# locuslab/icnn

Measured on AMD Instinct MI355X. Metric: inner-solves/sec (batch x iters), n=159 K=10, higher is better.
Workload: dtype f32 PICNN / f64 dual solve

## Files before the change

icnn_amd/_lib.py:

```python
import ctypes as C
import os

import torch

HERE = os.path.dirname(os.path.abspath(__file__))
LIB_PATH = os.path.join(HERE, "csrc", "libicnn_be.so")
if os.environ.get("ICNN_BE_LIB"):
    LIB_PATH = os.path.abspath(os.environ["ICNN_BE_LIB"])

ABI_VERSION = 12
MAX_LAYERS = 8
MAX_SLOTS = 31
MAX_ITERS = 64
MAX_ROUNDS = 128
VARIANT = {"dual": 0, "rl": 1, "pdipm": 2}
CUT_F32, CUT_F64 = 0, 1
ST_SINGULAR, ST_NONFINITE, ST_OVERFLOW, ST_UNFINISHED = 1, 2, 4, 8
ST_ERROR_MASK = ST_SINGULAR | ST_NONFINITE | ST_UNFINISHED | ST_OVERFLOW
FLAG_NO_CYCLE_SHORTCUT = 1
FLAG_TIME_SLICE = 2
FLAG_LOCKSTEP = 4
FLAG_TWO_KERNELS = 8
FLAG_PERSISTENT = 16
FLAG_F64_ENERGY = 32
FLAG_GLOBAL_BUNDLE = 64
FLAG_WAVE_PER_SAMPLE = 128
FLAG_MFMA_CONTRACTION = 256
FLAG_GENERIC_SHAPE = 512
SHAPE_INSTANCES = ["generic", "bibtex_kt16", "bibtex_kt32_grouped"]
LOSS = {"xent": 0, "mse": 1}
PATHS = ["ROWS", "TILE", "TILE_BUDGETED_THEN_ROWS", "ROUNDS_LOCKSTEP", "ROUNDS_SLICED_THEN_ROWS", "ROUNDS_SLICED_EXTRA"]
ADAM_KERNELS = ["NONE", "ROWS", "TILE"]
DUAL_KERNELS = ["small", "body", "wide"]
ERRORS = {-1: "ICNN_BE_EINVAL (bad argument)", -2: "ICNN_BE_ELIMIT (size beyond a compiled-in limit)",
          -3: "ICNN_BE_ELAUNCH (HIP launch failed)"}

EXPORTS = [
    "icnn_be_abi_version", "icnn_be_last_hip_error", "icnn_be_struct_size", "icnn_be_dual_lds_bytes", "icnn_be_bundle_capacity", "icnn_be_scratch_bytes",
    "icnn_be_state_init",
    "icnn_be_dual_step", "icnn_be_fc_pack_floats", "icnn_be_fc_pack", "icnn_be_fc_fg",
    "icnn_be_solve_fc", "icnn_be_solve_fc_reset", "icnn_be_conv_pack_floats", "icnn_be_conv_work_floats", "icnn_be_conv_pack", "icnn_be_conv_fg", "icnn_be_solve_conv",
    "icnn_be_implicit_feed", "icnn_be_export_active", "icnn_be_adam_workspace_bytes", "icnn_be_adam_fc", "icnn_be_adam_fc_obs",
    "icnn_be_adam_fc_each", "icnn_be_debug_adam_each_plan",
    "icnn_be_fc_context_work_floats", "icnn_be_fc_context", "icnn_be_fc_context_stage", "icnn_be_fc_context_norm", "icnn_be_fc_clamp",
    "icnn_be_conv_context_work_floats", "icnn_be_conv_context", "icnn_be_conv_clamp",
    "icnn_be_debug_profile", "icnn_be_debug_profile_fc", "icnn_be_debug_profile_conv", "icnn_be_debug_profile_phases",
    "icnn_be_debug_fast_math", "icnn_be_debug_trace", "icnn_be_debug_solve_plan", "icnn_be_debug_adam_plan", "icnn_be_debug_dual_plan",
    "icnn_be_debug_shape_instance", "icnn_be_debug_fc_deal",
    "icnn_be_fc_grad_floats", "icnn_be_fc_surrogate_grad_work_floats", "icnn_be_fc_surrogate_grad",
    "icnn_be_conv_grad_floats", "icnn_be_conv_surrogate_grad_work_floats", "icnn_be_conv_surrogate_grad",
    "icnn_be_fc_context_bn_work_floats", "icnn_be_fc_context_bn", "icnn_be_conv_context_bn_work_floats", "icnn_be_conv_context_bn",
# ... 639 lines not shown
```

icnn_amd/csrc/be_dual_dev.h:

```cpp
#pragma once
#include <hip/hip_runtime.h>
#include <math.h>
#include <type_traits>

#include "be_common.h"
#include "be_kernels.h"
#include "icnn_be.h"

namespace icnn_be {

namespace {

constexpr double BOUND_EPS = 1e-12;
constexpr double ARMIJO_ALPHA = 1e-5;
constexpr double GRAD_TOL = 1e-10;
constexpr double TINY = 1e-10;
constexpr double CYCLE_TOL = 1e-13;
constexpr double NOISE_TOL = 1e-10;
constexpr int NOISE_T0 = 12;
constexpr int ACCEL_T0 = 24;
constexpr int ACCEL_GAP = 6;
constexpr double ACCEL_NEG_RESID = 1e-10;
constexpr double ACCEL_D2MAX = 1e-3;
constexpr double ACCEL_RMAX = 0.98;
// ... 465 lines not shown
    }
#pragma unroll
    for (int p = KT - 1; p >= 0; --p) {
        if (p < k && ((fmask >> p) & 1ull)) {
            const double x = bcast(M[KT] * rinv, p);
            M[KT] = lane == p ? x : (lane < p ? M[KT] - M[p] * x : M[KT]);
        }
    }
    return StepResult{is_free ? M[KT] : 0.0, 1};
}

template <int I, int N, typename F>
__device__ __forceinline__ void static_for(F &&f) {
    if constexpr (I < N) {
        f(std::integral_constant<int, I>{});
        static_for<I + 1, N>(f);
    }
}
template <int P>
__device__ __forceinline__ double row_bcast(double v) {
    return __builtin_amdgcn_update_dpp(0.0, v, 0x150 + P, 0xf, 0xf, true);
}

template <int KS>
__device__ __noinline__ int inertia_not_above_dpp(const double *Hm_, int HP, int k, double mu) {
    static_assert(KS <= 16, "row broadcasts stay inside one 16-lane row");
    const int lane = lane_id();
    lds_cdouble *Hm = (lds_cdouble *)Hm_;
    HP = uni(HP); k = uni(k); mu = uni(mu);
    double M[KS];
#pragma unroll
    for (int j = 0; j < KS; ++j) M[j] = Hm[(lane < k ? lane : 0) * HP + (j < k ? j : 0)];
#pragma unroll
    for (int j = 0; j < KS; ++j) pin(M[j]);
#pragma unroll
    for (int j = 0; j < KS; ++j)
        M[j] = (lane < k && j < k) ? M[j] - (j == lane ? mu : 0.0) : (j == lane ? 1.0 : 0.0);
    double dp = 1.0;
    static_for<0, KS>([&](auto P) {
        constexpr int p = decltype(P)::value;
        const double d = row_bcast<p>(M[p]);
        dp = lane == p ? d : dp;
        const double nf = lane > p ? -(M[p] * rcp_nr(d)) : 0.0;
        static_for<p + 1, KS>([&](auto J) {
            constexpr int j = decltype(J)::value;
            M[j] = __builtin_fma(nf, row_bcast<p>(M[j]), M[j]);
        });
    });
    const unsigned long long nonpos = __ballot(lane < k && !(dp > 0.0));
    const unsigned long long zero = __ballot(lane < k && dp == 0.0);
    if (zero) {
        const int p0 = __builtin_ctzll(zero);
        return __popcll(nonpos & ((2ull << p0) - 1ull)) + (k - p0 - 1);
    }
    return __popcll(nonpos);
}

template <int KS, bool TRI = false>
__device__ __noinline__ StepResult newton_step_dpp(const double *Hm_, int HP, int k, int piv,
                                                   unsigned long long fmask, bool is_free, double g0) {
    static_assert(KS <= 16, "row broadcasts stay inside one 16-lane row");
    const int lane = lane_id();
    lds_cdouble *Hm = (lds_cdouble *)Hm_;
    HP = uni(HP); k = uni(k); piv = uni(piv); fmask = uni(fmask);
    double M[KS + 1];
    const int rl = lane < k ? lane : 0;
    auto at = [&](int i, int j) -> int {
        if (!TRI) return i * HP + j;
        const int c = i > j ? i : j, r = i > j ? j : i;
        return c * (c + 1) / 2 + r;
    };
    double h_ip = Hm[at(rl, piv)], h_pp = Hm[at(piv, piv)];
#pragma unroll
    for (int j = 0; j < KS; ++j) M[j] = Hm[at(rl, j < k ? j : 0)];
    pin(h_ip);
    pin(h_pp);
#pragma unroll
    for (int j = 0; j < KS; ++j) pin(M[j]);
    static_for<0, KS>([&](auto J) {
        constexpr int j = decltype(J)::value;
        double hv = ((M[j] - row_bcast<j>(h_ip)) - h_ip) + h_pp;
        pin(hv);
        const bool use = j < k && is_free && ((fmask >> j) & 1ull);
        M[j] = use ? hv : (j == lane ? 1.0 : 0.0);
    });
    M[KS] = is_free ? -g0 : 0.0;
    double rinv = 1.0;
    bool bad = false;
    static_for<0, KS>([&](auto P) {
        constexpr int p = decltype(P)::value;
        const double d = row_bcast<p>(M[p]);
        bad |= !(d != 0.0);
        const double inv = rcp_nr(d);
        rinv = lane == p ? inv : rinv;
        const double nf = lane > p ? -(M[p] * inv) : 0.0;
        static_for<p + 1, KS + 1>([&](auto J) {
            constexpr int j = decltype(J)::value;
            M[j] = __builtin_fma(nf, row_bcast<p>(M[j]), M[j]);
        });
        __builtin_amdgcn_sched_barrier(0);
    });
    if (__ballot(bad) & 0xffffull) return StepResult{0.0, 0};
    static_for<0, KS>([&](auto Q) {
        constexpr int p = KS - 1 - decltype(Q)::value;
        const double x = row_bcast<p>(M[KS] * rinv);
        M[KS] = lane == p ? x : (lane < p ? __builtin_fma(-M[p], x, M[KS]) : M[KS]);
    });
    return StepResult{is_free ? M[KS] : 0.0, 1};
}

__device__ __forceinline__ void swap16(double &x, double &y) {
    const auto lo = __builtin_amdgcn_permlane16_swap((unsigned)__double2loint(x), (unsigned)__double2loint(y), false, false);
    const auto hi = __builtin_amdgcn_permlane16_swap((unsigned)__double2hiint(x), (unsigned)__double2hiint(y), false, false);
    x = __hiloint2double((int)hi[0], (int)lo[0]);
    y = __hiloint2double((int)hi[1], (int)lo[1]);
}
__device__ __forceinline__ void swap32(double &x, double &y) {
    const auto lo = __builtin_amdgcn_permlane32_swap((unsigned)__double2loint(x), (unsigned)__double2loint(y), false, false);
    const auto hi = __builtin_amdgcn_permlane32_swap((unsigned)__double2hiint(x), (unsigned)__double2hiint(y), false, false);
    x = __hiloint2double((int)hi[0], (int)lo[0]);
    y = __hiloint2double((int)hi[1], (int)lo[1]);
}
template <int Q>
__device__ __forceinline__ double quarter_bcast(double v) {
    double a = v, b = v;
    swap16(a, b);
    double c = (Q & 1) ? b : a, d = c;
    swap32(c, d);
    return Q < 2 ? c : d;
}
__device__ __forceinline__ void quarter_gather(double v, double (&out)[4]) {
    double a = v, b = v;
// ... 123 lines not shown
            nf1 = quarter_bcast<qp>(i1 > p ? -(M1[sp] * inv) : 0.0);
        }
        static_for<sp, NS>([&](auto S) {
            constexpr int s = decltype(S)::value;
            const double pr = row_bcast<rp>(upper ? M1[s] : M0[s]);
            if constexpr (!upper) M0[s] = __builtin_fma(nf0, pr, M0[s]);
            M1[s] = __builtin_fma(nf1, pr, M1[s]);
        });
        __builtin_amdgcn_sched_barrier(0);
    });
    const bool own = (r & 3) == q;
    auto fold = [](unsigned long long m) -> unsigned { return (unsigned)((m | (m >> 16) | (m >> 32) | (m >> 48)) & 0xffffull); };
    unsigned nonpos = fold(__ballot(own && !(dp0 > 0.0))) | (fold(__ballot(own && !(dp1 > 0.0))) << 16);
    unsigned zero = fold(__ballot(own && dp0 == 0.0)) | (fold(__ballot(own && dp1 == 0.0)) << 16);
    const unsigned live = k >= 32 ? 0xffffffffu : ((1u << k) - 1u);
    nonpos &= live; zero &= live;
    if (zero) {
        const int p0 = __builtin_ctz(zero);
        return __popc(nonpos & ((2u << p0) - 1u)) + (k - p0 - 1);
    }
    return __popc(nonpos);
}

template <int KT>
__device__ __forceinline__ int inertia_not_above(const double *Hm, int HP, int k, double mu) {
    if (k <= 4) return inertia_not_above_dpp<4>(Hm, HP, k, mu);
    if (k <= 6) return inertia_not_above_dpp<6>(Hm, HP, k, mu);
    if (k <= 8) return inertia_not_above_dpp<8>(Hm, HP, k, mu);
    if (k <= 10) return inertia_not_above_dpp<10>(Hm, HP, k, mu);
    if (k <= 12) return inertia_not_above_dpp<12>(Hm, HP, k, mu);
    if (KT == 16 || k <= 16) return inertia_not_above_dpp<16>(Hm, HP, k, mu);
    if constexpr (KT > 16) {
        if (k <= 20) return inertia_not_above_2d<20>(Hm, HP, k, mu);
        if (k <= 24) return inertia_not_above_2d<24>(Hm, HP, k, mu);
        return inertia_not_above_2d<32>(Hm, HP, k, mu);
    }
    return 0;
}
__device__ __forceinline__ StepResult newton_step_tri(const double *P, int k, int piv, unsigned long long fmask, bool is_free,
                                                      double g0) {
    if (k <= 4) return newton_step_dpp<4, true>(P, 0, k, piv, fmask, is_free, g0);
    if (k <= 6) return newton_step_dpp<6, true>(P, 0, k, piv, fmask, is_free, g0);
    return newton_step_dpp<8, true>(P, 0, k, piv, fmask, is_free, g0);
}
template <int KT>
__device__ __forceinline__ StepResult newton_step(const double *Hm, int HP, int k, int piv, unsigned long long fmask,
                                                  bool is_free, double g0) {
    if (k <= 4) return newton_step_dpp<4>(Hm, HP, k, piv, fmask, is_free, g0);
    if (k <= 6) return newton_step_dpp<6>(Hm, HP, k, piv, fmask, is_free, g0);
    if (k <= 8) return newton_step_dpp<8>(Hm, HP, k, piv, fmask, is_free, g0);
    if (k <= 10) return newton_step_dpp<10>(Hm, HP, k, piv, fmask, is_free, g0);
    if (k <= 12) return newton_step_dpp<12>(Hm, HP, k, piv, fmask, is_free, g0);
    if (KT == 16 || k <= 16) return newton_step_dpp<16>(Hm, HP, k, piv, fmask, is_free, g0);
    if constexpr (KT > 16) {
        if (k <= 20) return newton_step_2d<20>(Hm, HP, k, piv, fmask, is_free, g0);
        if (k <= 24) return newton_step_2d<24>(Hm, HP, k, piv, fmask, is_free, g0);
        return newton_step_2d<32>(Hm, HP, k, piv, fmask, is_free, g0);
    }
    return StepResult{0.0, 0};
}

template <typename Op>
__device__ __forceinline__ double row16_reduce(double v, Op op) {
// ... 45 lines not shown
#pragma unroll
        for (int c = 0; c < NC; ++c) acc[c] += li * (double)As[i0 * ldA + jc[c]];
    }
#pragma unroll
    for (int c = 0; c < NC; ++c) fin(tid + c * nt, tid + c * nt < n_pad, acc[c]);
}
template <typename CutT, typename F>
__device__ __forceinline__ void for_columns(const CutT *As, int ldA, int k, int zrow, int n_pad, int nt, int tid,
                                            double lam, F &&fin) {
    const int per_thread = (n_pad + nt - 1) / nt;
    if (per_thread == 3) columns_nc<CutT, 3>(As, ldA, k, zrow, n_pad, nt, tid, lam, fin);
    else if (per_thread <= 2) columns_nc<CutT, 2>(As, ldA, k, zrow, n_pad, nt, tid, lam, fin);
    else if (per_thread == 4) columns_nc<CutT, 4>(As, ldA, k, zrow, n_pad, nt, tid, lam, fin);
    else
        for (int j0 = 0; j0 < n_pad; j0 += 4 * nt)
            columns_nc<CutT, 4>(As + j0, ldA, k, zrow, n_pad - j0, nt, tid, lam,
                                [&](int j, bool valid, double aj) { fin(j0 + j, valid, aj); });
}

#include "be_dual_valu_dev.h"
#include "be_ipm_dev.h"

template <typename CutT, int KT, int NW, bool RL, bool IPM = false, bool GLB = false, int LR = 0, bool SLICED = true,
          typename Shape = DynShape, typename ArgsT>
__device__ __forceinline__ void dual_step_body(const ArgsT &a, int u, int tid, unsigned char *smem, int round,
                                               int rows_cap, const CutT *crow_shared) {
    constexpr int NT = 64 * NW;
    const auto &st = a.st;
    const int lane = tid & 63, wave = tid >> 6;
    const bool w0 = wave == 0;
    auto wg_any = [&](bool p) -> bool { return NW == 1 ? (bool)__any(p) : (bool)__syncthreads_or(p); };
    auto combine = [&](double *Hm_, const double *Hp_, int HP_, int k_, int ncols) {
        if (NW == 1) return;
        sample_sync<NW>();
        for (int e = tid; e < k_ * ncols; e += NT) {
            const int r = e / ncols, c = e - r * ncols;
            double acc = 0.0;
            for (int w = 0; w < NW; ++w) acc += Hp_[(w * rows_cap + r) * HP_ + c];
            Hm_[r * HP_ + c] = acc;
        }
    };
    long long tick = ICNN_BE_PROF_ON(a.prof) ? (long long)__builtin_readcyclecounter() : 0;
    const int T = st.slots;
    const int TI = st.iters > 0 ? st.iters : T;
    const int finished_u = st.finished[u], t_raw = st.t_next[u], phase_u = st.phase[u], cnt_raw = st.count[u];
    const int slot_pre = tid < T ? st.active[(size_t)u * T + tid] : 0;
    const int slot_lane = NW == 1 ? slot_pre : (lane < T ? st.active[(size_t)u * T + lane] : 0);
    if (finished_u) return;
    const int t = __builtin_amdgcn_readfirstlane(t_raw);
    if (t >= TI) return;
    const bool resume = SLICED && __builtin_amdgcn_readfirstlane(phase_u) != 0;

    const int n = Shape::n(a), n_pad = Shape::n_pad(a), ldA = Shape::ldA(a);
    const auto &plan = Shape::plan(a);
    const int HP = (rows_cap + 1) | 1;
    static_assert(!IPM || !RL, "interior point is a variant of its own");
    const Carve cv = carve(KT, rows_cap, ldA, n_pad, (int)sizeof(CutT), plan.n_leaves, RL, NW, crow_shared == nullptr, IPM, GLB);
    const int cchunk = NW == 1 ? n_pad : (((n_pad / 16 + NW - 1) / NW) * 16);
    const int cbeg = wave * cchunk < n_pad ? wave * cchunk : n_pad;
    const int cend = cbeg + cchunk < n_pad ? cbeg + cchunk : n_pad;
    CutT *As = GLB ? static_cast<CutT *>(st.scratch) + (size_t)u * (st.slots + 2) * ldA : reinterpret_cast<CutT *>(smem + cv.As);
    static_assert(LR == 0 || GLB, "split staging belongs to the device-memory rounds");
    CutT *AsL = reinterpret_cast<CutT *>(smem + ((cv.total + 15) & ~15));
    const bool mirror = LR > 0 && rows_cap <= HV_KMAX;
    double *zs = reinterpret_cast<double *>(smem + cv.zs);
    double *ws = reinterpret_cast<double *>(smem + cv.ws);
    double *sp = reinterpret_cast<double *>(smem + cv.sp);
    double *Hm = reinterpret_cast<double *>(smem + cv.Hm);
    double *Hp = reinterpret_cast<double *>(smem + cv.Hp) + (NW == 1 ? 0 : wave * rows_cap * HP);
    double *Hp0 = reinterpret_cast<double *>(smem + cv.Hp);
    double *leaf = Hm;
    double *psum = Hm + KT * plan.n_leaves;
    int *slots = reinterpret_cast<int *>(smem + cv.ints);

    const CutT *g_row = static_cast<const CutT *>(a.g) + (size_t)u * n;
    const double f_u = (sizeof(CutT) == 4 && (st.flags & ICNN_BE_FLAG_F64_ENERGY))
                           ? static_cast<const double *>(a.f)[u] : (double)static_cast<const CutT *>(a.f)[u];
    double *y_row = st.y + (size_t)u * n;
    CutT *G_u = static_cast<CutT *>(st.G) + (size_t)u * T * n;
// ... 145 lines not shown
            h_u[slot_new] = h_new;
            if (st.fvals) st.fvals[(size_t)u * T + slot_new] = f_u;
        }
        if (wg_any(bad)) {
            if (tid == 0) { st.status[u] |= ICNN_BE_ST_NONFINITE; st.finished[u] = 1; st.skip_fg[u] = 1; }
            return;
        }
    } else {
        for (int j = tid; j < n_pad; j += NT) {
            const CutT v = j < n ? G_u[(size_t)slot_new * n + j] : (CutT)0;
            As[cnt * ldA + j] = v;
            if (LR > 0 && mirror && cnt < LR) AsL[cnt * ldA + j] = v;
        }
        h_new = h_u[slot_new];
        stage_older();
    }
    lap(0);
    const CutT *crow = crow_shared ? crow_shared : As + rows_cap * ldA;
    if (!crow_shared)
        for (int j = tid; j < ldA; j += NT) { As[rows_cap * ldA + j] = (CutT)0; As[(rows_cap + 1) * ldA + j] = (CutT)1; }
    const double h_i = lane < cnt ? h_old : h_new;
    const bool hv_on = !(st.flags & ICNN_BE_FLAG_MFMA_CONTRACTION);
    const int hv_p = hv_pitch(k);
    const bool valu = hv_on && (NW > 1 || (n_pad <= 192 && sizeof(CutT) == 4 && k <= HV_K1MAX)) && !RL && !IPM && k >= 2 &&
                      k <= HV_KMAX && (LR == 0 || mirror) && n_pad <= 256 * NW && NW * hv_p <= n_pad;
    double *hv_part = zs;
    const HvEntry hv_first = hv_entry<true>(lane, k, HP);
    sample_sync<NW>();

    lap(1);
    if (!RL && !resume) {
        bool deficient = false;
        const double cfac = (double)(k > n ? k : n) * Cut<CutT>::eps;
        if (k == 1) {
            bool nz = false;
            for (int j = tid; j < n; j += NT) nz |= As[j] != (CutT)0;
            deficient = !wg_any(nz);
        } else if (sizeof(CutT) == 8 && NW == 1) {
            for (int sweep = 0; sweep < 30; ++sweep) {
                bool rotated = false;
                for (int p = 0; p < k - 1; ++p)
                    for (int q = p + 1; q < k; ++q) {
                        double al = 0, be = 0, ga = 0;
                        for (int j = lane; j < n; j += 64) {
                            const double vp = (double)As[p * ldA + j], vq = (double)As[q * ldA + j];
                            al += vp * vp; be += vq * vq; ga += vp * vq;
                        }
// ... 8 lines not shown
                            const double vp = (double)As[p * ldA + j], vq = (double)As[q * ldA + j];
                            As[p * ldA + j] = (CutT)(c * vp - s * vq);
                            As[q * ldA + j] = (CutT)(s * vp + c * vq);
                        }
                    }
                if (!rotated) break;
            }
            double sv = 0.0, smax = 0.0;
            for (int r = 0; r < k; ++r) {
                double ss = 0;
                for (int j = lane; j < n; j += 64) { const double v = (double)As[r * ldA + j]; ss += v * v; }
                ss = sqrt(wave_sum(ss));
                if (lane == r) sv = ss;
                smax = fmax(smax, ss);
            }
            deficient = __popcll(__ballot(lane < k && sv > smax * cfac)) < k;
            sample_sync<NW>();
            for (int r = 0; r < k; ++r) {
                const CutT *src = r < cnt ? G_u + (size_t)slots[r] * n : g_row;
                for (int j = lane; j < n_pad; j += 64) As[r * ldA + j] = j < n ? src[j] : (CutT)0;
            }
            sample_sync<NW>();
        } else {
            if (valu) {
                hv_column_pass_k<CutT, NW, false, LR, GLB, (NW == 1 && KT > 16)>(As, AsL, ldA, k, rows_cap, n, n_pad, tid, 0.0, hv_part + wave * hv_p);
                sample_sync<NW>();
                hv_gather<NW, false>(hv_part, hv_p, Hm, HP, k, tid, NT, hv_entry<false>(tid, k, HP));
            } else {
                contract_mfma<CutT, KT, false>(As, ldA, k, crow, cbeg, cend, ws, zs, Hp, HP);
                combine(Hm, Hp0, HP, k, k);
            }
            sample_sync<NW>();
            double trace = 0, total = 0, dmax = 0, rmax = 0;
            {
                double diag = 0, rsum = 0, rabs = 0;
                if (lane < k) {
                    diag = Hm[lane * HP + lane];
                    for (int c = 0; c < k; ++c) { const double v = Hm[lane * HP + c]; rsum += v; rabs += fabs(v); }
                }
                for (int i = 0; i < k; ++i) {
                    const double di = bcast(diag, i);
                    trace += di; dmax = fmax(dmax, di);
                    total += bcast(rsum, i); rmax = fmax(rmax, bcast(rabs, i));
                }
            }
            const double lo = fmax(dmax, total / (double)k);
            const double hi = fmin(trace, rmax);
            const double c2 = cfac * cfac;
            if (inertia_not_above<KT>(Hm, HP, k, c2 * hi) == 0) {
                deficient = false;
            } else if (inertia_not_above<KT>(Hm, HP, k, c2 * lo) > 0) {
                deficient = true;
            } else {
                jacobi_lane0<KT, NW>(Hm, HP, k, tid);
                const double ev = lane < k ? fmax(Hm[lane * HP + lane], 0.0) : 0.0;
                const double svv = sqrt(ev), smax = wave_max(svv);
                deficient = __popcll(__ballot(lane < k && svv > smax * cfac)) < k;
            }
            sample_sync<NW>();
        }
        if (deficient) {
            if (tid == 0) { st.finished[u] = 1; st.n_iters[u] = t - 1; st.skip_fg[u] = 1; }
            return;
        }
    }

    lap(2);
    double lam = 0.0;
    int updates = 0, updates_before = 0;
    if constexpr (IPM) {
        int ipm_status = 0;
        if constexpr (NW > 1) {
            const int kp = k < 2 ? 2 : hv_padded(k);
            const bool waves_ok = sizeof(CutT) == 4 && k <= IPM_KMAX_WAVES && NW * ((ipm_nv(kp) + 3) & ~3) <= n_pad;
// ... 29 lines not shown
        const int backoff_cap = RL ? 10 : 50;
        const bool shortcut = !(st.flags & ICNN_BE_FLAG_NO_CYCLE_SHORTCUT);
        lam = lane < k ? 1.0 / (double)k : 0.0;
        double prev1 = 0.0, prev2 = 0.0, prev3 = 0.0, prev4 = 0.0;
        int hist = 0, last_jump = -1000;
        double d4_prev = -1.0;
        bool abort_sample = false, parked = false;
        int upd0 = 0;
        double *park = st.park + (size_t)u * (5 * T + 4);
        if (resume) {
            updates = upd0 = updates_before = uni((int)park[5 * T]);
            hist = uni((int)park[5 * T + 1]);
            last_jump = uni((int)park[5 * T + 2]);
            d4_prev = uni(park[5 * T + 3]);
            if (lane < k) {
                lam = park[lane]; prev1 = park[T + lane]; prev2 = park[2 * T + lane]; prev3 = park[3 * T + lane];
                prev4 = park[4 * T + lane];
            }
        }
        int budget = a.budget > 0 ? a.budget : cap;

        while (updates < cap) {
            if (SLICED && budget-- <= 0) { parked = true; break; }
            if (valu) {
                double *part = hv_part + (updates & 1) * (NW * hv_p);
                hv_column_pass_k<CutT, NW, true, LR, GLB, (NW == 1 && KT > 16)>(As, AsL, ldA, k, rows_cap, n, n_pad, tid, lam, part + wave * hv_p);
                sample_sync<NW>();
                lap(4);
                if (NW > 1) hv_gather<NW, true>(part, hv_p, Hp, HP, k, lane, 64, hv_first);
                lap(5);
            } else {
                for_columns<CutT>(As, ldA, k, rows_cap, n_pad, NT, tid, lam, [&](int j, bool valid, double aj) {
                    double z = sigmoid_fast(aj);
                    double w = z * (1.0 - z);
                    if (j >= n) { z = 0.0; w = 0.0; }
                    if (valid) {
                        zs[j] = z;
                        ws[j] = w;
                        if (RL) sp[j] = j < n ? softplus_fast(aj) : 0.0;
                    }
                });
                sample_sync<NW>();
                lap(4);
                contract_mfma<CutT, KT, true>(As, ldA, k, crow, cbeg, cend, ws, zs, Hp, HP, lap);
                combine(Hm, Hp0, HP, k, k + 1);
                sample_sync<NW>();
                lap(5);
            }
            const double *Hq = valu ? Hp : Hm;
            static_assert(HV_K1MAX <= 8 && hv_padded(HV_K1MAX) == HV_K1MAX, "the packed triangle of a k-cut bundle is the k-cut instance's");
            const bool tri = NW == 1 && valu;
            const int hvT = k * (k + 1) / 2;

            const double grad = lane < k ? -c_i + (tri ? hv_part[(updates & 1) * (NW * hv_p) + hvT + lane] : Hq[lane * HP + k]) : 0.0;
            int piv_v = 0;
            {
                const double mx = rows_reduce<KT>(lane < k ? lam : -1e300, k, [](double x, double y) { return fmax(x, y); });
                const unsigned long long at = __ballot(lane < k && lam == mx);
                piv_v = at ? __builtin_ctzll(at) : 0;
            }
            const int piv = __builtin_amdgcn_readfirstlane(piv_v);
            const bool is_piv = lane == piv;
            const double red = is_piv ? 1.0 : lam;
            const double keep = is_piv ? 0.0 : 1.0;
            const double g0 = grad - keep * bcast(grad, piv);
            const bool bound = is_piv || (red <= BOUND_EPS && g0 > 0.0);
            const bool is_free = lane < k && !bound;
            const unsigned long long fmask = __ballot(is_free);
            const double nrm2 = rows_reduce<KT>(is_free ? g0 * g0 : 0.0, k, [](double x, double y) { return x + y; });
            if (sqrt(nrm2) < GRAD_TOL) break;

            lap(8);
            const StepResult sr = tri ? newton_step_tri(hv_part + (updates & 1) * (NW * hv_p), k, piv, fmask, is_free, g0)
                                      : newton_step<KT>(Hq, HP, k, piv, fmask, is_free, g0);
            const double step = sr.step;
            if (!__builtin_amdgcn_readfirstlane(sr.ok)) {
                if (tid == 0) st.status[u] |= ICNN_BE_ST_SINGULAR;
                if (!RL) abort_sample = true;
                break;
            }

            lap(9);
            double tt = 1.0;
            double fval = 0.0, slope = 0.0;
            if (RL) {
                double dmax = 0.0;
                for (int i = 0; i < k; ++i) dmax = fmax(dmax, fabs(bcast(step, i)));
                tt = fmin(1.0 / dmax, 1.0);
                sample_sync<NW>();
                np_pairwise_rows<NW, double>(plan, 1, [&](int, int j) { return sp[j]; }, leaf, psum, tid);
                double cl = 0.0;
                for (int i = 0; i < k; ++i) { cl += bcast(c_i * lam, i); slope += bcast(step * g0, i); }
                fval = -cl + psum[0];
                sample_sync<NW>();
            }
            double lam_new = lam;
// ... 219 lines not shown
```

icnn_amd/csrc/be_dual_valu_dev.h:

```cpp
#pragma once

constexpr int HV_KMAX = 20;
__host__ __device__ constexpr int hv_cap(int K) { return K <= 12 ? 40 : (K <= 16 ? 24 : 16); }
__host__ __device__ constexpr int hv_wcol(int e) {
    int c = 0;
    while ((c + 1) * (c + 2) / 2 <= e) ++c;
    return c;
}
__host__ __device__ constexpr int hv_wrow(int e) { return e - hv_wcol(e) * (hv_wcol(e) + 1) / 2; }
__host__ __device__ constexpr int hv_nv(int K, bool hess) { return K * (K + 1) / 2 + (hess ? K : 0); }
__host__ __device__ constexpr int hv_chunk_len(int nv, int cap) { return (nv + (nv + cap - 1) / cap - 1) / ((nv + cap - 1) / cap); }
__host__ __device__ constexpr int hv_padded(int k) { return k <= 7 ? k : (k + 1) & ~1; }
__host__ __device__ constexpr int hv_pitch(int k) { return (hv_nv(hv_padded(k), true) + 3) & ~3; }
__host__ __device__ constexpr int hv_count(int nv, int level) {
    int c = nv;
    for (int l = 0; l < level; ++l) c = (c + 1) / 2;
    return c;
}

__device__ __forceinline__ void hv_swap32(double &x, double &y) {
    const auto lo = __builtin_amdgcn_permlane32_swap((unsigned)__double2loint(x), (unsigned)__double2loint(y), false, false);
    const auto hi = __builtin_amdgcn_permlane32_swap((unsigned)__double2hiint(x), (unsigned)__double2hiint(y), false, false);
    x = __hiloint2double((int)hi[0], (int)lo[0]);
    y = __hiloint2double((int)hi[1], (int)lo[1]);
// ... 128 lines not shown
        for (int c = 0; c < NC; ++c) {
            z[c] = sigmoid_fast(acc[c]);
            w[c] = z[c] * (1.0 - z[c]);
        }
    }
#pragma unroll
    for (int c = 0; c < NC; ++c)
        if (tid + c * NT >= n) { z[c] = 0.0; w[c] = 0.0; }
    if (KR != K) asm volatile("" ::: "memory");
    hv_chunks<CutT, K, NC, 0, hv_chunk_len(NV, hv_cap(K)), NV, HESS, KR>(av, load, z, w, lane, Pw);
}

template <typename CutT, int K, int NW, bool HESS, int LR, bool GSRC>
__device__ __noinline__ void hv_column_pass_fn(const CutT *As_, const CutT *AsL_, int ldA, int k, int zrow, int n, int n_pad,
                                               int tid, double lam, double *Pw_) {
    typedef const __attribute__((address_space(3))) CutT *LdsCut;
    typedef const __attribute__((address_space(1))) CutT *GlbCut;
    typedef __attribute__((address_space(3))) double *LdsDbl;
    ldA = uni(ldA); k = uni(k); zrow = uni(zrow); n = uni(n); n_pad = uni(n_pad);
    if constexpr (GSRC) hv_column_pass<CutT, K, NW, HESS, LR>((GlbCut)As_, (LdsCut)AsL_, ldA, k, zrow, n, n_pad, tid, lam, (LdsDbl)Pw_);
    else hv_column_pass<CutT, K, NW, HESS, LR>((LdsCut)As_, (LdsCut)AsL_, ldA, k, zrow, n, n_pad, tid, lam, (LdsDbl)Pw_);
}

template <typename CutT, int NW, bool HESS, int LR, bool GSRC, bool ALLFN = false>
__device__ __forceinline__ void hv_column_pass_k(const CutT *As, const CutT *AsL, int ldA, int k, int zrow, int n, int n_pad,
                                                 int tid, double lam, double *Pw) {
    if constexpr (ALLFN) {
        switch (hv_padded(k)) {
        case 2: hv_column_pass_fn<CutT, 2, NW, HESS, LR, GSRC>(As, AsL, ldA, k, zrow, n, n_pad, tid, lam, Pw); break;
        case 3: hv_column_pass_fn<CutT, 3, NW, HESS, LR, GSRC>(As, AsL, ldA, k, zrow, n, n_pad, tid, lam, Pw); break;
        case 4: hv_column_pass_fn<CutT, 4, NW, HESS, LR, GSRC>(As, AsL, ldA, k, zrow, n, n_pad, tid, lam, Pw); break;
        case 5: hv_column_pass_fn<CutT, 5, NW, HESS, LR, GSRC>(As, AsL, ldA, k, zrow, n, n_pad, tid, lam, Pw); break;
        case 6: hv_column_pass_fn<CutT, 6, NW, HESS, LR, GSRC>(As, AsL, ldA, k, zrow, n, n_pad, tid, lam, Pw); break;
        case 7: hv_column_pass_fn<CutT, 7, NW, HESS, LR, GSRC>(As, AsL, ldA, k, zrow, n, n_pad, tid, lam, Pw); break;
        default: hv_column_pass_fn<CutT, 8, NW, HESS, LR, GSRC>(As, AsL, ldA, k, zrow, n, n_pad, tid, lam, Pw); break;
        }
        return;
    }
    switch (hv_padded(k)) {
    case 2: hv_column_pass<CutT, 2, NW, HESS, LR>(As, AsL, ldA, k, zrow, n, n_pad, tid, lam, Pw); break;
    case 3: hv_column_pass<CutT, 3, NW, HESS, LR>(As, AsL, ldA, k, zrow, n, n_pad, tid, lam, Pw); break;
    case 4: hv_column_pass<CutT, 4, NW, HESS, LR>(As, AsL, ldA, k, zrow, n, n_pad, tid, lam, Pw); break;
    case 5: hv_column_pass<CutT, 5, NW, HESS, LR>(As, AsL, ldA, k, zrow, n, n_pad, tid, lam, Pw); break;
    case 6: hv_column_pass<CutT, 6, NW, HESS, LR>(As, AsL, ldA, k, zrow, n, n_pad, tid, lam, Pw); break;
    case 7: hv_column_pass<CutT, 7, NW, HESS, LR>(As, AsL, ldA, k, zrow, n, n_pad, tid, lam, Pw); break;
    case 8: hv_column_pass_fn<CutT, 8, NW, HESS, LR, GSRC>(As, AsL, ldA, k, zrow, n, n_pad, tid, lam, Pw); break;
    case 10: hv_column_pass_fn<CutT, 10, NW, HESS, LR, GSRC>(As, AsL, ldA, k, zrow, n, n_pad, tid, lam, Pw); break;
    case 12: hv_column_pass_fn<CutT, 12, NW, HESS, LR, GSRC>(As, AsL, ldA, k, zrow, n, n_pad, tid, lam, Pw); break;
    case 14: hv_column_pass_fn<CutT, 14, NW, HESS, LR, GSRC>(As, AsL, ldA, k, zrow, n, n_pad, tid, lam, Pw); break;
// ... 70 lines not shown
```

icnn_amd/csrc/be_fused.hip:

```cpp
#include "be_dual_dev.h"
#include "be_dual_small_dev.h"
#include "be_picnn_fc_dev.h"
#include "be_picnn_fc_rows_dev.h"

namespace icnn_be {

namespace {

static_assert(NWAVE == TM, "one wave per sample in the dual phase");

struct FusedArgs {
    DualArgs da;
    FcArgs fa;
    int rounds, crow_off, samples_off, sample_bytes;
    int grouped;
    int group_cap, need_off;
    long long *trace;
    SolveReset reset;
};
typedef const __attribute__((address_space(4))) FusedArgs KArgs;

__device__ __forceinline__ void reset_sample(const icnn_be_state &st, const SolveReset &rs, int u, int lane) {
    const int n = st.n;
    double *yr = st.y + (size_t)u * n;
    if (rs.y0) {
        const double *src = rs.y0 + (size_t)u * n;
        for (int j = lane; j < n; j += 64) yr[j] = src[j];
    } else {
        for (int j = lane; j < n; j += 64) yr[j] = rs.fill;
    }
    if (lane == 0) {
        st.count[u] = 0;
        st.finished[u] = 0;
        st.status[u] = 0;
        st.n_iters[u] = st.iters > 0 ? st.iters : st.slots;
        st.newton_iters[u] = 0;
        st.t_next[u] = 0;
        st.phase[u] = 0;
        st.skip_fg[u] = 0;
    }
}

template <bool RL, int KT, bool IPM = false, bool SLICED = false, typename Shape = DynShape, int GROUPED = -1>
__global__ __launch_bounds__(NTHREADS) void fused_fc_solve_kernel(FusedArgs args) {
    extern __shared__ __attribute__((aligned(16))) unsigned char smem[];
    KArgs *kp0 = (KArgs *)__builtin_amdgcn_kernarg_segment_ptr();
    {
        const int ldA = Shape::ldA(args.da);
        float *crow = reinterpret_cast<float *>(smem + args.crow_off);
        for (int j = thread_id(); j < 2 * ldA; j += NTHREADS) crow[j] = j < ldA ? 0.f : 1.f;
        if ((GROUPED < 0 ? args.grouped != 0 : GROUPED != 0) && thread_id() < TM)
            reinterpret_cast<int *>(smem + args.need_off)[TM + thread_id()] = 0;
    }
    if (args.reset.on) {
        const int wave = uni(thread_id() >> 6), u = blockIdx.x * args.fa.tile_rows + wave;
        if (wave < args.fa.tile_rows && u < args.da.st.batch) reset_sample(args.da.st, args.reset, u, thread_id() & 63);
        __syncthreads();
    }
    const int rounds = args.rounds;
    for (int r = 0; r < rounds; ++r) {
        KArgs *kp = kp0;
        int tile = blockIdx.x;
        asm volatile("" : "+s"(kp), "+s"(tile));
        fc_fg_tile<Shape>(kp->fa, tile, reinterpret_cast<float *>(smem));
        __syncthreads();
        int wave = uni(thread_id() >> 6), round = r;
        asm volatile("" : "+s"(kp), "+s"(tile), "+s"(wave), "+s"(round));
        KArgs &k = *kp;
        const int u = tile * k.fa.tile_rows + wave;
        const bool mine = wave < k.fa.tile_rows && u < k.da.st.batch;
        if (GROUPED < 0 ? !k.grouped : GROUPED == 0) {
            if (mine) {
                const int rows_cap = round + 1 < k.da.st.slots ? round + 1 : k.da.st.slots;
                dual_step_body<float, KT, 1, RL, IPM, false, 0, SLICED, Shape>(k.da, u, thread_id() & 63,
                                                                        smem + k.samples_off + wave * k.sample_bytes, round, rows_cap,
                                                                        reinterpret_cast<const float *>(smem + k.crow_off));
            }
            __syncthreads();
            continue;
        }
        int *need = reinterpret_cast<int *>(smem + k.need_off);
        int kk = 0;
        if (mine && k.da.st.finished[u] == 0 && k.da.st.t_next[u] < k.rounds) kk = k.da.st.count[u] + 1;
        kk = uni(kk);
        if (kk > k.da.st.slots) kk = k.da.st.slots;
        if ((thread_id() & 63) == 0)
            need[wave] = kk > 0 ? (carve(KT, kk, Shape::ldA(k.da), Shape::n_pad(k.da), 4, Shape::plan(k.da).n_leaves, RL, 1, false, IPM).total + 15) & ~15 : 0;
        __syncthreads();
        int g = 0, off = 0, my_g = 0, my_off = 0;
        for (int i = 0; i < TM; ++i) {
            const int nb = need[i];
            if (off + nb > k.group_cap) { ++g; off = 0; }
            if (i == wave) { my_g = g; my_off = off; }
            off += nb;
        }
        my_g = uni(my_g); my_off = uni(my_off);
        int alive = kk > 0;
        int *done = need + TM;
        long long tq = ICNN_BE_PROF_ON(k.da.prof) ? (long long)__builtin_readcyclecounter() : 0;
// ... 280 lines not shown
hipError_t launch_fused_fc_solve(const icnn_be_fc_model &m, const float *ctx, const icnn_be_state &st, float *f_work,
                                 float *g_work, long long *dual_prof, hipStream_t stream, int tile_rows, int budget,
                                 const SolveReset &reset) {
    if (budget > 0 && reset.on) return hipErrorInvalidValue;
    FusedTileLayout lay;
    if (!fused_tile_layout(m, st, tile_rows, budget, lay)) return hipErrorInvalidValue;
    FusedArgs args{};
    int fg_bytes = 0;
    if (fill_args(m, args.fa, fg_bytes) != 0) return hipErrorInvalidValue;
    args.fa.ctx = ctx; args.fa.y = st.y; args.fa.f = f_work; args.fa.g = g_work; args.fa.finished = st.skip_fg;
    args.fa.batch = st.batch; args.fa.prof = fc_profile_buffer(); args.fa.tile_rows = tile_rows;
    if (!make_dual_args(args.da, st, f_work, g_work, 0, budget, st.slots, dual_prof)) return hipErrorInvalidValue;
    args.rounds = st.iters > 0 ? st.iters : st.slots;
    args.crow_off = lay.crow_off; args.samples_off = 0; args.sample_bytes = lay.sample_bytes;
    args.grouped = lay.grouped; args.group_cap = lay.group_cap; args.need_off = lay.need_off;
    args.trace = dual_trace_buffer();
    args.reset = reset;
    const bool rl = st.variant == ICNN_BE_VARIANT_RL, big = st.slots > 15;
    auto kern = big ? (rl ? fused_fc_solve_kernel<true, 32> : fused_fc_solve_kernel<false, 32>)
                    : (rl ? fused_fc_solve_kernel<true, 16> : fused_fc_solve_kernel<false, 16>);
    if (st.variant == ICNN_BE_VARIANT_PDIPM) kern = big ? fused_fc_solve_kernel<false, 32, true> : fused_fc_solve_kernel<false, 16, true>;
    if (budget > 0) kern = big ? fused_fc_solve_kernel<false, 32, false, true> : fused_fc_solve_kernel<false, 16, false, true>;
    switch (pick_shape_instance(args, lay)) {
    case ICNN_BE_SHAPE_BIBTEX_KT16: kern = fused_fc_solve_kernel<false, 16, false, false, BibtexShape, 0>; break;
    case ICNN_BE_SHAPE_BIBTEX_KT32_GROUPED: kern = fused_fc_solve_kernel<false, 32, false, false, BibtexShape, 1>; break;
    default: break;
    }
    return launch_kernel(kern, dim3((st.batch + tile_rows - 1) / tile_rows), dim3(NTHREADS), lay.lds, stream, args);
}

}
```

include/icnn_be.h:

```cpp
#ifndef ICNN_BE_H
#define ICNN_BE_H

#include <stddef.h>

#ifdef __cplusplus
extern "C" {
#endif

#if defined(__GNUC__)
#define ICNN_BE_API __attribute__((visibility("default")))
#else
#define ICNN_BE_API
#endif

#define ICNN_BE_ABI_VERSION 12
#define ICNN_BE_MAX_LAYERS 8
#define ICNN_BE_MAX_SLOTS 31
#define ICNN_BE_MAX_ITERS 64
#define ICNN_BE_MAX_ROUNDS 128

#define ICNN_BE_VARIANT_DUAL 0
#define ICNN_BE_VARIANT_RL 1
#define ICNN_BE_VARIANT_PDIPM 2

// ... 16 lines not shown

#define ICNN_BE_ADAM_NONE 0
#define ICNN_BE_ADAM_ROWS 1
#define ICNN_BE_ADAM_TILE 2

#define ICNN_BE_DUAL_PLAN_SMALL 0
#define ICNN_BE_DUAL_PLAN_BODY 1
#define ICNN_BE_DUAL_PLAN_WIDE 2

#define ICNN_BE_EINVAL (-1)
#define ICNN_BE_ELIMIT (-2)
#define ICNN_BE_ELAUNCH (-3)

#define ICNN_BE_FLAG_NO_CYCLE_SHORTCUT 1
#define ICNN_BE_FLAG_TIME_SLICE 2
#define ICNN_BE_FLAG_LOCKSTEP 4
#define ICNN_BE_FLAG_TWO_KERNELS 8
#define ICNN_BE_FLAG_PERSISTENT 16

#define ICNN_BE_FLAG_WAVE_PER_SAMPLE 128
#define ICNN_BE_FLAG_MFMA_CONTRACTION 256
#define ICNN_BE_FLAG_GLOBAL_BUNDLE 64
#define ICNN_BE_FLAG_GENERIC_SHAPE 512
#define ICNN_BE_FLAG_F64_ENERGY 32

typedef struct icnn_be_state {
    int batch;
    int n;
    int slots;
    int cut_dtype;
    int variant;
    int flags;
    double *y;
    void *G;
    double *h;
    double *ys;
    double *lam;
    int *active;
    int *count;
    int *n_iters;
    int *finished;
    int *status;
    int *newton_iters;
    int *t_next;
    int *phase;
    int *skip_fg;
// ... 689 lines not shown
```

Baseline: 46.11 million.

## Specialize early dual rounds with capped bundle size and inlined DPP solvers

For the bibtex 16-slot ungrouped dual instance, the first HV_K1MAX rounds (where at most eight cuts exist) now run a separate dual_step_body instantiation capped at eight cuts. This instantiation always takes the fused VALU Hessian pass, dispatches only over the small column-pass sizes, and uses force-inlined copies of the DPP inertia and Newton-step routines instead of noinline calls. The aim is to remove call overhead and the generic dispatch branches in early rounds. The cost is a larger kernel with two body instances, which can raise register pressure and instruction-cache footprint. A new flag disables the path.

```diff
diff --git a/icnn_amd/_lib.py b/icnn_amd/_lib.py
--- a/icnn_amd/_lib.py
+++ b/icnn_amd/_lib.py
@@ -27,6 +27,7 @@
 FLAG_WAVE_PER_SAMPLE = 128
 FLAG_MFMA_CONTRACTION = 256
 FLAG_GENERIC_SHAPE = 512
+FLAG_NO_ROUND_CLASSES = 1024
 SHAPE_INSTANCES = ["generic", "bibtex_kt16", "bibtex_kt32_grouped"]
 LOSS = {"xent": 0, "mse": 1}
 PATHS = ["ROWS", "TILE", "TILE_BUDGETED_THEN_ROWS", "ROUNDS_LOCKSTEP", "ROUNDS_SLICED_THEN_ROWS", "ROUNDS_SLICED_EXTRA"]
diff --git a/icnn_amd/csrc/be_dual_dev.h b/icnn_amd/csrc/be_dual_dev.h
--- a/icnn_amd/csrc/be_dual_dev.h
+++ b/icnn_amd/csrc/be_dual_dev.h
@@ -511,92 +511,16 @@
     return __builtin_amdgcn_update_dpp(0.0, v, 0x150 + P, 0xf, 0xf, true);
 }
 
-template <int KS>
-__device__ __noinline__ int inertia_not_above_dpp(const double *Hm_, int HP, int k, double mu) {
-    static_assert(KS <= 16, "row broadcasts stay inside one 16-lane row");
-    const int lane = lane_id();
-    lds_cdouble *Hm = (lds_cdouble *)Hm_;
-    HP = uni(HP); k = uni(k); mu = uni(mu);
-    double M[KS];
-#pragma unroll
-    for (int j = 0; j < KS; ++j) M[j] = Hm[(lane < k ? lane : 0) * HP + (j < k ? j : 0)];
-#pragma unroll
-    for (int j = 0; j < KS; ++j) pin(M[j]);
-#pragma unroll
-    for (int j = 0; j < KS; ++j)
-        M[j] = (lane < k && j < k) ? M[j] - (j == lane ? mu : 0.0) : (j == lane ? 1.0 : 0.0);
-    double dp = 1.0;
-    static_for<0, KS>([&](auto P) {
-        constexpr int p = decltype(P)::value;
-        const double d = row_bcast<p>(M[p]);
-        dp = lane == p ? d : dp;
-        const double nf = lane > p ? -(M[p] * rcp_nr(d)) : 0.0;
-        static_for<p + 1, KS>([&](auto J) {
-            constexpr int j = decltype(J)::value;
-            M[j] = __builtin_fma(nf, row_bcast<p>(M[j]), M[j]);
-        });
-    });
-    const unsigned long long nonpos = __ballot(lane < k && !(dp > 0.0));
-    const unsigned long long zero = __ballot(lane < k && dp == 0.0);
-    if (zero) {
-        const int p0 = __builtin_ctzll(zero);
-        return __popcll(nonpos & ((2ull << p0) - 1ull)) + (k - p0 - 1);
-    }
-    return __popcll(nonpos);
-}
-
-template <int KS, bool TRI = false>
-__device__ __noinline__ StepResult newton_step_dpp(const double *Hm_, int HP, int k, int piv,
-                                                   unsigned long long fmask, bool is_free, double g0) {
-    static_assert(KS <= 16, "row broadcasts stay inside one 16-lane row");
-    const int lane = lane_id();
-    lds_cdouble *Hm = (lds_cdouble *)Hm_;
-    HP = uni(HP); k = uni(k); piv = uni(piv); fmask = uni(fmask);
-    double M[KS + 1];
-    const int rl = lane < k ? lane : 0;
-    auto at = [&](int i, int j) -> int {
-        if (!TRI) return i * HP + j;
-        const int c = i > j ? i : j, r = i > j ? j : i;
-        return c * (c + 1) / 2 + r;
-    };
-    double h_ip = Hm[at(rl, piv)], h_pp = Hm[at(piv, piv)];
-#pragma unroll
-    for (int j = 0; j < KS; ++j) M[j] = Hm[at(rl, j < k ? j : 0)];
-    pin(h_ip);
-    pin(h_pp);
-#pragma unroll
-    for (int j = 0; j < KS; ++j) pin(M[j]);
-    static_for<0, KS>([&](auto J) {
-        constexpr int j = decltype(J)::value;
-        double hv = ((M[j] - row_bcast<j>(h_ip)) - h_ip) + h_pp;
-        pin(hv);
-        const bool use = j < k && is_free && ((fmask >> j) & 1ull);
-        M[j] = use ? hv : (j == lane ? 1.0 : 0.0);
-    });
-    M[KS] = is_free ? -g0 : 0.0;
-    double rinv = 1.0;
-    bool bad = false;
-    static_for<0, KS>([&](auto P) {
-        constexpr int p = decltype(P)::value;
-        const double d = row_bcast<p>(M[p]);
-        bad |= !(d != 0.0);
-        const double inv = rcp_nr(d);
-        rinv = lane == p ? inv : rinv;
-        const double nf = lane > p ? -(M[p] * inv) : 0.0;
-        static_for<p + 1, KS + 1>([&](auto J) {
-            constexpr int j = decltype(J)::value;
-            M[j] = __builtin_fma(nf, row_bcast<p>(M[j]), M[j]);
-        });
-        __builtin_amdgcn_sched_barrier(0);
-    });
-    if (__ballot(bad) & 0xffffull) return StepResult{0.0, 0};
-    static_for<0, KS>([&](auto Q) {
-        constexpr int p = KS - 1 - decltype(Q)::value;
-        const double x = row_bcast<p>(M[KS] * rinv);
-        M[KS] = lane == p ? x : (lane < p ? __builtin_fma(-M[p], x, M[KS]) : M[KS]);
-    });
-    return StepResult{is_free ? M[KS] : 0.0, 1};
-}
+#define DPP_ROWS_ATTR __noinline__
+#define DPP_ROWS_NAME(f) f
+#include "be_dual_dpp_rows.h"
+#undef DPP_ROWS_ATTR
+#undef DPP_ROWS_NAME
+#define DPP_ROWS_ATTR __forceinline__
+#define DPP_ROWS_NAME(f) f##_inl
+#include "be_dual_dpp_rows.h"
+#undef DPP_ROWS_ATTR
+#undef DPP_ROWS_NAME
 
 __device__ __forceinline__ void swap16(double &x, double &y) {
     const auto lo = __builtin_amdgcn_permlane16_swap((unsigned)__double2loint(x), (unsigned)__double2loint(y), false, false);
@@ -766,8 +690,14 @@
     return __popc(nonpos);
 }
 
-template <int KT>
+template <int KT, int KCAP = 0>
 __device__ __forceinline__ int inertia_not_above(const double *Hm, int HP, int k, double mu) {
+    if constexpr (KCAP > 0) {
+        static_assert(KCAP <= 8, "capped bodies hold bundles of up to eight cuts");
+        if (KCAP <= 4 || k <= 4) return inertia_not_above_dpp_inl<4>(Hm, HP, k, mu);
+        if (KCAP <= 6 || k <= 6) return inertia_not_above_dpp_inl<6>(Hm, HP, k, mu);
+        return inertia_not_above_dpp_inl<8>(Hm, HP, k, mu);
+    }
     if (k <= 4) return inertia_not_above_dpp<4>(Hm, HP, k, mu);
     if (k <= 6) return inertia_not_above_dpp<6>(Hm, HP, k, mu);
     if (k <= 8) return inertia_not_above_dpp<8>(Hm, HP, k, mu);
@@ -781,8 +711,14 @@
     }
     return 0;
 }
+template <int KCAP = 0>
 __device__ __forceinline__ StepResult newton_step_tri(const double *P, int k, int piv, unsigned long long fmask, bool is_free,
                                                       double g0) {
+    if constexpr (KCAP > 0) {
+        if (KCAP <= 4 || k <= 4) return newton_step_dpp_inl<4, true>(P, 0, k, piv, fmask, is_free, g0);
+        if (KCAP <= 6 || k <= 6) return newton_step_dpp_inl<6, true>(P, 0, k, piv, fmask, is_free, g0);
+        return newton_step_dpp_inl<8, true>(P, 0, k, piv, fmask, is_free, g0);
+    }
     if (k <= 4) return newton_step_dpp<4, true>(P, 0, k, piv, fmask, is_free, g0);
     if (k <= 6) return newton_step_dpp<6, true>(P, 0, k, piv, fmask, is_free, g0);
     return newton_step_dpp<8, true>(P, 0, k, piv, fmask, is_free, g0);
@@ -874,7 +810,7 @@
 #include "be_ipm_dev.h"
 
 template <typename CutT, int KT, int NW, bool RL, bool IPM = false, bool GLB = false, int LR = 0, bool SLICED = true,
-          typename Shape = DynShape, typename ArgsT>
+          typename Shape = DynShape, int KCAP = 0, typename ArgsT>
 __device__ __forceinline__ void dual_step_body(const ArgsT &a, int u, int tid, unsigned char *smem, int round,
                                                int rows_cap, const CutT *crow_shared) {
     constexpr int NT = 64 * NW;
@@ -907,6 +843,11 @@
     const auto &plan = Shape::plan(a);
     const int HP = (rows_cap + 1) | 1;
     static_assert(!IPM || !RL, "interior point is a variant of its own");
+    if constexpr (KCAP > 0) {
+        static_assert(NW == 1 && KT == 16 && !RL && !IPM && !GLB && LR == 0 && sizeof(CutT) == 4, "capped bodies: one-wave dual variant");
+        static_assert(KCAP <= HV_K1MAX && Shape::FIXED && Shape::N_PAD <= 192 && hv_pitch(KCAP) <= Shape::N_PAD,
+                      "every bundle of a capped body takes the fused VALU pass");
+    }
     const Carve cv = carve(KT, rows_cap, ldA, n_pad, (int)sizeof(CutT), plan.n_leaves, RL, NW, crow_shared == nullptr, IPM, GLB);
     const int cchunk = NW == 1 ? n_pad : (((n_pad / 16 + NW - 1) / NW) * 16);
     const int cbeg = wave * cchunk < n_pad ? wave * cchunk : n_pad;
@@ -1098,7 +1039,7 @@
     const double h_i = lane < cnt ? h_old : h_new;
     const bool hv_on = !(st.flags & ICNN_BE_FLAG_MFMA_CONTRACTION);
     const int hv_p = hv_pitch(k);
-    const bool valu = hv_on && (NW > 1 || (n_pad <= 192 && sizeof(CutT) == 4 && k <= HV_K1MAX)) && !RL && !IPM && k >= 2 &&
+    const bool valu = KCAP > 0 ? k >= 2 : hv_on && (NW > 1 || (n_pad <= 192 && sizeof(CutT) == 4 && k <= HV_K1MAX)) && !RL && !IPM && k >= 2 &&
                       k <= HV_KMAX && (LR == 0 || mirror) && n_pad <= 256 * NW && NW * hv_p <= n_pad;
     double *hv_part = zs;
     const HvEntry hv_first = hv_entry<true>(lane, k, HP);
@@ -1153,8 +1094,8 @@
             }
             sample_sync<NW>();
         } else {
-            if (valu) {
-                hv_column_pass_k<CutT, NW, false, LR, GLB, (NW == 1 && KT > 16)>(As, AsL, ldA, k, rows_cap, n, n_pad, tid, 0.0, hv_part + wave * hv_p);
+            if (KCAP > 0 || valu) {
+                hv_column_pass_k<CutT, NW, false, LR, GLB, (NW == 1 && KT > 16), KCAP>(As, AsL, ldA, k, rows_cap, n, n_pad, tid, 0.0, hv_part + wave * hv_p);
                 sample_sync<NW>();
                 hv_gather<NW, false>(hv_part, hv_p, Hm, HP, k, tid, NT, hv_entry<false>(tid, k, HP));
             } else {
@@ -1178,9 +1119,9 @@
             const double lo = fmax(dmax, total / (double)k);
             const double hi = fmin(trace, rmax);
             const double c2 = cfac * cfac;
-            if (inertia_not_above<KT>(Hm, HP, k, c2 * hi) == 0) {
+            if (inertia_not_above<KT, KCAP>(Hm, HP, k, c2 * hi) == 0) {
                 deficient = false;
-            } else if (inertia_not_above<KT>(Hm, HP, k, c2 * lo) > 0) {
+            } else if (inertia_not_above<KT, KCAP>(Hm, HP, k, c2 * lo) > 0) {
                 deficient = true;
             } else {
                 jacobi_lane0<KT, NW>(Hm, HP, k, tid);
@@ -1256,9 +1197,9 @@
 
         while (updates < cap) {
             if (SLICED && budget-- <= 0) { parked = true; break; }
-            if (valu) {
+            if (KCAP > 0 || valu) {
                 double *part = hv_part + (updates & 1) * (NW * hv_p);
-                hv_column_pass_k<CutT, NW, true, LR, GLB, (NW == 1 && KT > 16)>(As, AsL, ldA, k, rows_cap, n, n_pad, tid, lam, part + wave * hv_p);
+                hv_column_pass_k<CutT, NW, true, LR, GLB, (NW == 1 && KT > 16), KCAP>(As, AsL, ldA, k, rows_cap, n, n_pad, tid, lam, part + wave * hv_p);
                 sample_sync<NW>();
                 lap(4);
                 if (NW > 1) hv_gather<NW, true>(part, hv_p, Hp, HP, k, lane, 64, hv_first);
@@ -1283,7 +1224,7 @@
             }
             const double *Hq = valu ? Hp : Hm;
             static_assert(HV_K1MAX <= 8 && hv_padded(HV_K1MAX) == HV_K1MAX, "the packed triangle of a k-cut bundle is the k-cut instance's");
-            const bool tri = NW == 1 && valu;
+            const bool tri = KCAP > 0 || (NW == 1 && valu);
             const int hvT = k * (k + 1) / 2;
 
             const double grad = lane < k ? -c_i + (tri ? hv_part[(updates & 1) * (NW * hv_p) + hvT + lane] : Hq[lane * HP + k]) : 0.0;
@@ -1305,7 +1246,7 @@
             if (sqrt(nrm2) < GRAD_TOL) break;
 
             lap(8);
-            const StepResult sr = tri ? newton_step_tri(hv_part + (updates & 1) * (NW * hv_p), k, piv, fmask, is_free, g0)
+            const StepResult sr = tri ? newton_step_tri<KCAP>(hv_part + (updates & 1) * (NW * hv_p), k, piv, fmask, is_free, g0)
                                       : newton_step<KT>(Hq, HP, k, piv, fmask, is_free, g0);
             const double step = sr.step;
             if (!__builtin_amdgcn_readfirstlane(sr.ok)) {
diff --git a/icnn_amd/csrc/be_dual_dpp_rows.h b/icnn_amd/csrc/be_dual_dpp_rows.h
--- /dev/null
+++ b/icnn_amd/csrc/be_dual_dpp_rows.h
@@ -0,0 +1,86 @@
+template <int KS>
+__device__ DPP_ROWS_ATTR int DPP_ROWS_NAME(inertia_not_above_dpp)(const double *Hm_, int HP, int k, double mu) {
+    static_assert(KS <= 16, "row broadcasts stay inside one 16-lane row");
+    const int lane = lane_id();
+    lds_cdouble *Hm = (lds_cdouble *)Hm_;
+    HP = uni(HP); k = uni(k); mu = uni(mu);
+    double M[KS];
+#pragma unroll
+    for (int j = 0; j < KS; ++j) M[j] = Hm[(lane < k ? lane : 0) * HP + (j < k ? j : 0)];
+#pragma unroll
+    for (int j = 0; j < KS; ++j) pin(M[j]);
+#pragma unroll
+    for (int j = 0; j < KS; ++j)
+        M[j] = (lane < k && j < k) ? M[j] - (j == lane ? mu : 0.0) : (j == lane ? 1.0 : 0.0);
+    double dp = 1.0;
+    static_for<0, KS>([&](auto P) {
+        constexpr int p = decltype(P)::value;
+        const double d = row_bcast<p>(M[p]);
+        dp = lane == p ? d : dp;
+        const double nf = lane > p ? -(M[p] * rcp_nr(d)) : 0.0;
+        static_for<p + 1, KS>([&](auto J) {
+            constexpr int j = decltype(J)::value;
+            M[j] = __builtin_fma(nf, row_bcast<p>(M[j]), M[j]);
+        });
+    });
+    const unsigned long long nonpos = __ballot(lane < k && !(dp > 0.0));
+    const unsigned long long zero = __ballot(lane < k && dp == 0.0);
+    if (zero) {
+        const int p0 = __builtin_ctzll(zero);
+        return __popcll(nonpos & ((2ull << p0) - 1ull)) + (k - p0 - 1);
+    }
+    return __popcll(nonpos);
+}
+
+template <int KS, bool TRI = false>
+__device__ DPP_ROWS_ATTR StepResult DPP_ROWS_NAME(newton_step_dpp)(const double *Hm_, int HP, int k, int piv,
+                                                                  unsigned long long fmask, bool is_free, double g0) {
+    static_assert(KS <= 16, "row broadcasts stay inside one 16-lane row");
+    const int lane = lane_id();
+    lds_cdouble *Hm = (lds_cdouble *)Hm_;
+    HP = uni(HP); k = uni(k); piv = uni(piv); fmask = uni(fmask);
+    double M[KS + 1];
+    const int rl = lane < k ? lane : 0;
+    auto at = [&](int i, int j) -> int {
+        if (!TRI) return i * HP + j;
+        const int c = i > j ? i : j, r = i > j ? j : i;
+        return c * (c + 1) / 2 + r;
+    };
+    double h_ip = Hm[at(rl, piv)], h_pp = Hm[at(piv, piv)];
+#pragma unroll
+    for (int j = 0; j < KS; ++j) M[j] = Hm[at(rl, j < k ? j : 0)];
+    pin(h_ip);
+    pin(h_pp);
+#pragma unroll
+    for (int j = 0; j < KS; ++j) pin(M[j]);
+    static_for<0, KS>([&](auto J) {
+        constexpr int j = decltype(J)::value;
+        double hv = ((M[j] - row_bcast<j>(h_ip)) - h_ip) + h_pp;
+        pin(hv);
+        const bool use = j < k && is_free && ((fmask >> j) & 1ull);
+        M[j] = use ? hv : (j == lane ? 1.0 : 0.0);
+    });
+    M[KS] = is_free ? -g0 : 0.0;
+    double rinv = 1.0;
+    bool bad = false;
+    static_for<0, KS>([&](auto P) {
+        constexpr int p = decltype(P)::value;
+        const double d = row_bcast<p>(M[p]);
+        bad |= !(d != 0.0);
+        const double inv = rcp_nr(d);
+        rinv = lane == p ? inv : rinv;
+        const double nf = lane > p ? -(M[p] * inv) : 0.0;
+        static_for<p + 1, KS + 1>([&](auto J) {
+            constexpr int j = decltype(J)::value;
+            M[j] = __builtin_fma(nf, row_bcast<p>(M[j]), M[j]);
+        });
+        __builtin_amdgcn_sched_barrier(0);
+    });
+    if (__ballot(bad) & 0xffffull) return StepResult{0.0, 0};
+    static_for<0, KS>([&](auto Q) {
+        constexpr int p = KS - 1 - decltype(Q)::value;
+        const double x = row_bcast<p>(M[KS] * rinv);
+        M[KS] = lane == p ? x : (lane < p ? __builtin_fma(-M[p], x, M[KS]) : M[KS]);
+    });
+    return StepResult{is_free ? M[KS] : 0.0, 1};
+}
diff --git a/icnn_amd/csrc/be_dual_valu_dev.h b/icnn_amd/csrc/be_dual_valu_dev.h
--- a/icnn_amd/csrc/be_dual_valu_dev.h
+++ b/icnn_amd/csrc/be_dual_valu_dev.h
@@ -174,9 +174,24 @@
     else hv_column_pass<CutT, K, NW, HESS, LR>((LdsCut)As_, (LdsCut)AsL_, ldA, k, zrow, n, n_pad, tid, lam, (LdsDbl)Pw_);
 }
 
-template <typename CutT, int NW, bool HESS, int LR, bool GSRC, bool ALLFN = false>
+template <typename CutT, int K, int KCAP, int NW, bool HESS, int LR>
+__device__ __forceinline__ void hv_column_pass_upto(const CutT *As, const CutT *AsL, int ldA, int k, int zrow, int n, int n_pad,
+                                                    int tid, double lam, double *Pw) {
+    if constexpr (K >= KCAP) {
+        hv_column_pass<CutT, K, NW, HESS, LR>(As, AsL, ldA, k, zrow, n, n_pad, tid, lam, Pw);
+    } else {
+        if (hv_padded(k) <= K) hv_column_pass<CutT, K, NW, HESS, LR>(As, AsL, ldA, k, zrow, n, n_pad, tid, lam, Pw);
+        else hv_column_pass_upto<CutT, K + 1, KCAP, NW, HESS, LR>(As, AsL, ldA, k, zrow, n, n_pad, tid, lam, Pw);
+    }
+}
+template <typename CutT, int NW, bool HESS, int LR, bool GSRC, bool ALLFN = false, int KCAP = 0>
 __device__ __forceinline__ void hv_column_pass_k(const CutT *As, const CutT *AsL, int ldA, int k, int zrow, int n, int n_pad,
                                                  int tid, double lam, double *Pw) {
+    if constexpr (KCAP > 0) {
+        static_assert(KCAP <= HV_K1MAX && hv_padded(KCAP) == KCAP && !ALLFN, "capped bodies: bundles of up to eight cuts");
+        hv_column_pass_upto<CutT, 2, KCAP, NW, HESS, LR>(As, AsL, ldA, k, zrow, n, n_pad, tid, lam, Pw);
+        return;
+    }
     if constexpr (ALLFN) {
         switch (hv_padded(k)) {
         case 2: hv_column_pass_fn<CutT, 2, NW, HESS, LR, GSRC>(As, AsL, ldA, k, zrow, n, n_pad, tid, lam, Pw); break;
diff --git a/icnn_amd/csrc/be_fused.hip b/icnn_amd/csrc/be_fused.hip
--- a/icnn_amd/csrc/be_fused.hip
+++ b/icnn_amd/csrc/be_fused.hip
@@ -8,6 +8,8 @@
 namespace {
 
 static_assert(NWAVE == TM, "one wave per sample in the dual phase");
+
+constexpr int ROUND_CLASS_CAP = HV_K1MAX;
 
 struct FusedArgs {
     DualArgs da;
@@ -41,8 +43,9 @@
     }
 }
 
-template <bool RL, int KT, bool IPM = false, bool SLICED = false, typename Shape = DynShape, int GROUPED = -1>
+template <bool RL, int KT, bool IPM = false, bool SLICED = false, typename Shape = DynShape, int GROUPED = -1, bool CLASSES = false>
 __global__ __launch_bounds__(NTHREADS) void fused_fc_solve_kernel(FusedArgs args) {
+    static_assert(!CLASSES || (GROUPED == 0 && KT == 16 && !RL && !IPM && !SLICED), "round classes: the ungrouped 16-slot dual instance");
     extern __shared__ __attribute__((aligned(16))) unsigned char smem[];
     KArgs *kp0 = (KArgs *)__builtin_amdgcn_kernarg_segment_ptr();
     {
@@ -72,9 +75,13 @@
         if (GROUPED < 0 ? !k.grouped : GROUPED == 0) {
             if (mine) {
                 const int rows_cap = round + 1 < k.da.st.slots ? round + 1 : k.da.st.slots;
-                dual_step_body<float, KT, 1, RL, IPM, false, 0, SLICED, Shape>(k.da, u, thread_id() & 63,
-                                                                        smem + k.samples_off + wave * k.sample_bytes, round, rows_cap,
-                                                                        reinterpret_cast<const float *>(smem + k.crow_off));
+                unsigned char *region = smem + k.samples_off + wave * k.sample_bytes;
+                const float *crow = reinterpret_cast<const float *>(smem + k.crow_off);
+                if (CLASSES && round < ROUND_CLASS_CAP)
+                    dual_step_body<float, KT, 1, RL, IPM, false, 0, SLICED, Shape, CLASSES ? ROUND_CLASS_CAP : 0>(
+                        k.da, u, thread_id() & 63, region, round, rows_cap, crow);
+                else
+                    dual_step_body<float, KT, 1, RL, IPM, false, 0, SLICED, Shape>(k.da, u, thread_id() & 63, region, round, rows_cap, crow);
             }
             __syncthreads();
             continue;
@@ -401,7 +408,11 @@
     if (st.variant == ICNN_BE_VARIANT_PDIPM) kern = big ? fused_fc_solve_kernel<false, 32, true> : fused_fc_solve_kernel<false, 16, true>;
     if (budget > 0) kern = big ? fused_fc_solve_kernel<false, 32, false, true> : fused_fc_solve_kernel<false, 16, false, true>;
     switch (pick_shape_instance(args, lay)) {
-    case ICNN_BE_SHAPE_BIBTEX_KT16: kern = fused_fc_solve_kernel<false, 16, false, false, BibtexShape, 0>; break;
+    case ICNN_BE_SHAPE_BIBTEX_KT16:
+        kern = (st.flags & (ICNN_BE_FLAG_NO_ROUND_CLASSES | ICNN_BE_FLAG_MFMA_CONTRACTION))
+                   ? fused_fc_solve_kernel<false, 16, false, false, BibtexShape, 0>
+                   : fused_fc_solve_kernel<false, 16, false, false, BibtexShape, 0, true>;
+        break;
     case ICNN_BE_SHAPE_BIBTEX_KT32_GROUPED: kern = fused_fc_solve_kernel<false, 32, false, false, BibtexShape, 1>; break;
     default: break;
     }
diff --git a/include/icnn_be.h b/include/icnn_be.h
--- a/include/icnn_be.h
+++ b/include/icnn_be.h
@@ -62,6 +62,7 @@
 #define ICNN_BE_FLAG_MFMA_CONTRACTION 256
 #define ICNN_BE_FLAG_GLOBAL_BUNDLE 64
 #define ICNN_BE_FLAG_GENERIC_SHAPE 512
+#define ICNN_BE_FLAG_NO_ROUND_CLASSES 1024
 #define ICNN_BE_FLAG_F64_ENERGY 32
 
 typedef struct icnn_be_state {
```

Result: faster. 47.77 million (median of 6 runs) (+3.6%).
